# cgranerob/Land-Surface-Temperature-Super-Resolution-with-a-Scale-Invariance-Free-Neural-Approach

Hardware: AMD Instinct MI355X
Metric: LST+NDVI 256x256 patches/sec (train fwd+bwd), whole job (higher is better)
Workload: dtype f32; 1 GPU; ModelB SIF-NN-SR2 (gradFTM loss) batch 64/GPU, synthetic 256x256, 1x MI355X, fwd+loss+bwd+Adam; batch_per_gpu=64, patch=256x256 (LST 64x64 + NDVI 256x256), parallelism=dp1, loss=sr2

## Files before the change

land-surface-temperature-super-resolution-with-a-scale-invariance-free-neural-approach_amd/csrc/bn.hip:

```cpp
#include "edge_conv.h"

namespace {

template <int NT>
static __device__ __forceinline__ void block_sum2(double& s1, double& s2, double (*wsum)[2]) {
#pragma unroll
  for (int m = 32; m > 0; m >>= 1) { s1 += __shfl_xor(s1, m); s2 += __shfl_xor(s2, m); }
  const int lane = threadIdx.x & 63, wave = threadIdx.x >> 6;
  if (lane == 0) { wsum[wave][0] = s1; wsum[wave][1] = s2; }
  __syncthreads();
  s1 = 0.0; s2 = 0.0;
#pragma unroll
  for (int w = 0; w < NT / 64; ++w) { s1 += wsum[w][0]; s2 += wsum[w][1]; }
}

static __device__ __forceinline__ float mul2_add(float a, float b, float c, float d) {
#pragma clang fp contract(off)
  const float p = a * b, q = c * d;
  return p + q;
}

__global__ __launch_bounds__(256) void bn_finalize_kernel(const float* __restrict__ partials, int nblk, int C,
                                                          double count, const float* __restrict__ gamma,
                                                          const float* __restrict__ beta, float* run_mean,
// ... 173 lines not shown
      double t = 0.0;
      for (int g = 0; g < 64; ++g) t += part[g][el];
      xs_out[e] = poisoned != 0 ? __uint_as_float(0x7fc00000u) : (float)t;
    }
    return;
  }
  double s1 = 0.0, s2 = 0.0;
  for (int k = tid; k < nblk; k += 256) {
    const float2 v = *reinterpret_cast<const float2*>(partials + ((size_t)k * C + c) * 2);
    s1 += (double)v.x; s2 += (double)v.y;
  }
  block_sum2<256>(s1, s2, wsum);
  if (tid == 0) {
    const double db = s1, dg = s2;
    dbeta[c] = (float)db;
    dgamma[c] = (float)dg;
    write_coef<FROZEN>(coef, C, c, scale, mean, invstd, db, dg, count);
    write_coef_f<FROZEN>(coef_f, C, c, scale, shift, invstd, beta, db, dg, count);
    if (poisoned != 0) poison_channel(dgamma, dbeta, coef, coef_f, C, c);
  }
}

template <int NT, bool FROZEN>
__global__ __launch_bounds__(NT) void bn_bwd_finalize2_kernel(const float* __restrict__ pa, int na,
                                                               const float* __restrict__ pb, int nb, int C, double count,
                                                               const float* __restrict__ scale,
                                                               const float* __restrict__ mean,
                                                               const float* __restrict__ invstd, float* dgamma,
                                                               float* dbeta, double* coef, const float* __restrict__ shift,
                                                               const float* __restrict__ beta, float* coef_f, const int* nf) {
  SIFSR_CHAIN_PRIO();
  __shared__ double wsum[NT / 64][2];
  const int c = blockIdx.x, tid = threadIdx.x;
  const int poisoned = nf != nullptr ? nf[NF_BATCH] : 0;
  double s1 = 0.0, s2 = 0.0;
  for (int k = tid; k < na; k += NT) { const float2 v = *reinterpret_cast<const float2*>(pa + ((size_t)k * C + c) * 2); s1 += (double)v.x; s2 += (double)v.y; }
  for (int k = tid; k < nb; k += NT) { const float2 v = *reinterpret_cast<const float2*>(pb + ((size_t)k * C + c) * 2); s1 += (double)v.x; s2 += (double)v.y; }
  block_sum2<NT>(s1, s2, wsum);
  if (tid == 0) {
    const double db = s1;
    const double dg = (double)invstd[c] * (s2 - (double)mean[c] * db);
    dbeta[c] = (float)db;
    dgamma[c] = (float)dg;
    write_coef<FROZEN>(coef, C, c, scale, mean, invstd, db, dg, count);
    write_coef_f<FROZEN>(coef_f, C, c, scale, shift, invstd, beta, db, dg, count);
    if (poisoned != 0) poison_channel(dgamma, dbeta, coef, coef_f, C, c);
  }
}

template <int C, bool HS>
__global__ __launch_bounds__(256) void bn_bwd_apply_kernel(const float* __restrict__ g, const float* __restrict__ y,
                                                           const float* __restrict__ scale,
                                                           const float* __restrict__ shift,
                                                           const double* __restrict__ coef,
                                                           size_t nquads, float* __restrict__ dy, const PoolAdj pa) {
  SIFSR_CHAIN_PRIO();
  constexpr int Q = C / 4;
  const int c4 = threadIdx.x % Q;
  const float4 sc = ld4(scale + 4 * c4), sh = ld4(shift + 4 * c4);
  double sd[4], k1[4], k0[4];
// ... 65 lines not shown
    default: return SIFSR_ERR_SHAPE;
  }
  SIFSR_LAUNCH_CHECK();
  return SIFSR_OK;
}

int launch_bn_bwd_finalize(const float* partials, int nblk, int C, double count, const float* scale, const float* mean,
                           const float* invstd, float* dgamma, float* dbeta, double* coef, hipStream_t s, const float* shift,
                           const float* beta, float* coef_f, const float* xs_partials, int xs_n, float* xs_out, int frozen,
                           const int* nf) {
  if (coef_f != nullptr && (!shift || !beta)) return SIFSR_ERR_ARG;
  if (xs_partials != nullptr && (xs_n < 1 || !xs_out)) return SIFSR_ERR_ARG;
  const int extra = xs_partials != nullptr ? (xs_n + 3) / 4 : 0;
  if (frozen)
    hipLaunchKernelGGL(bn_bwd_finalize_kernel<true>, dim3(C + extra), dim3(256), 0, s, partials, nblk, C, count, scale, mean, invstd,
                       dgamma, dbeta, coef, shift, beta, coef_f, xs_partials, xs_n, xs_out, nf);
  else
    hipLaunchKernelGGL(bn_bwd_finalize_kernel<false>, dim3(C + extra), dim3(256), 0, s, partials, nblk, C, count, scale, mean, invstd,
                       dgamma, dbeta, coef, shift, beta, coef_f, xs_partials, xs_n, xs_out, nf);
  SIFSR_LAUNCH_CHECK();
  return SIFSR_OK;
}

int launch_bn_bwd_finalize2(const float* pa, int na, const float* pb, int nb, int C, double count, const float* scale,
                            const float* mean, const float* invstd, float* dgamma, float* dbeta, double* coef, hipStream_t s,
                            const float* shift, const float* beta, float* coef_f, int frozen, const int* nf) {
  if (coef_f != nullptr && (!shift || !beta)) return SIFSR_ERR_ARG;
#define BN_FIN2(NT_, FR_) hipLaunchKernelGGL((bn_bwd_finalize2_kernel<NT_, FR_>), dim3(C), dim3(NT_), 0, s, pa, na, pb, nb, C, count, scale, mean, \
                                             invstd, dgamma, dbeta, coef, shift, beta, coef_f, nf)
  if (na + nb > 4096) { if (frozen) BN_FIN2(1024, true); else BN_FIN2(1024, false); }
  else { if (frozen) BN_FIN2(256, true); else BN_FIN2(256, false); }
#undef BN_FIN2
  SIFSR_LAUNCH_CHECK();
  return SIFSR_OK;
}

int launch_bn_bwd_apply(const float* g, const float* y, const float* scale, const float* shift, const double* coef,
                        int C, size_t npix, float* dy, hipStream_t s, const float* gp, int H, int W) {
  if (gp != nullptr && (H < 2 || W < 2 || H % 2 || W % 2 || npix % ((size_t)H * W))) return SIFSR_ERR_SHAPE;
  const PoolAdj pa{gp, H, W};
  const size_t nquads = npix * (size_t)C / 4;
  size_t blocks = (nquads + 255) / 256;
  if (blocks > 8192) blocks = 8192;
  const bool hs = sifsr_half_storage();
#define BN_APPLY(C_, HS_) hipLaunchKernelGGL((bn_bwd_apply_kernel<C_, HS_>), dim3((int)blocks), dim3(256), 0, s, g, y, scale, shift, coef, nquads, dy, pa)
  switch (C) {
    case 16: if (hs) BN_APPLY(16, true); else BN_APPLY(16, false); break;
    case 32: if (hs) BN_APPLY(32, true); else BN_APPLY(32, false); break;
    case 64: if (hs) BN_APPLY(64, true); else BN_APPLY(64, false); break;
    default: return SIFSR_ERR_SHAPE;
  }
// ... 11 lines not shown
```

land-surface-temperature-super-resolution-with-a-scale-invariance-free-neural-approach_amd/csrc/edge_conv.h:

```cpp
#pragma once
#include "common.h"

int conv_in_fwd_blocks(int B, int H, int W);
int launch_conv_in_fwd(const float* x, const float* w, float* y, float* partials, int B, int H, int W, hipStream_t s,
                       int* nf_image = nullptr);
int launch_conv_in_wgrad(const float* x, const float* dy, float* partials, int nblk, float* dw, int B, int H, int W, hipStream_t s);
int launch_conv_out_fwd(const float* y, const float* scale, const float* shift, const float* w, const float* bias,
                        float* out, int B, int H, int W, hipStream_t s,
                        const int* nf = nullptr);
int launch_conv_out_dgrad(const float* dsr, const float* w, float* g, int B, int H, int W, hipStream_t s);
int launch_conv_out_wgrad(const float* y, const float* scale, const float* shift, const float* dsr, float* partials,
                          int nblk, float* dw, float* db, int B, int H, int W, hipStream_t s);
int launch_conv_in_wgrad_fused(const float* x, const float* g, const float* y, const float* scale, const float* shift,
                               const double* coef, float* partials, int nblk, float* dw, int B, int H, int W, hipStream_t s);
size_t conv_in_gram_scratch_floats();
int launch_conv_in_gram(const float* x, float* scratch, int B, int H, int W, hipStream_t s);
const double* conv_in_gram_result(const float* scratch);
int launch_conv_in_dz_wgrad(const float* x, const float* dz, float* partials, int nblk, int B, int H, int W, hipStream_t s);
int launch_conv_in_dw_combine(const float* partials, int nblk, const double* gram, const float* w, const double* coef, float* dw,
                              hipStream_t s);
int launch_tail_bwd_reduce(const float* y, const float* scale, const float* shift, const float* mean, const float* invstd,
                           const float* dsr, const float* w, float* wpart, float* bnpart, int nblk, int B, int H, int W,
                           hipStream_t s, int* nf = nullptr);
int launch_tail_bwd_apply(const float* y, const float* scale, const float* shift, const double* coef, const float* dsr,
                          const float* w, float* dy, int B, int H, int W, hipStream_t s);
int launch_sum_partials(const float* partials, int nblk, int n, float* out, hipStream_t s);

int launch_bn_finalize(const float* partials, int nblk, int C, double count, const float* gamma, const float* beta,
                       float* run_mean, float* run_var, float momentum, float eps, float* mean, float* invstd,
                       float* scale, float* shift, hipStream_t s,
                       int* nf = nullptr);
int launch_bn_eval_coeffs(const float* params, const float* running, float eps, float* scale, float* shift, hipStream_t s,
                          int* nf = nullptr, const int* nf_pack = nullptr);
int launch_bn_bwd_reduce(const float* g, const float* y, const float* scale, const float* shift, const float* mean,
                         const float* invstd, int C, size_t npix, float* partials, int nblk, hipStream_t s,
                         const float* gp = nullptr, int H = 0, int W = 0, float* g_out = nullptr);
int launch_bn_bwd_finalize(const float* partials, int nblk, int C, double count, const float* scale, const float* mean,
                           const float* invstd, float* dgamma, float* dbeta, double* coef, hipStream_t s,
                           const float* shift = nullptr, const float* beta = nullptr, float* coef_f = nullptr,
                           const float* xs_partials = nullptr, int xs_n = 0, float* xs_out = nullptr,
                           int frozen = 0,
                           const int* nf = nullptr);
int launch_bn_bwd_finalize2(const float* pa, int na, const float* pb, int nb, int C, double count, const float* scale,
                            const float* mean, const float* invstd, float* dgamma, float* dbeta, double* coef, hipStream_t s,
                            const float* shift = nullptr, const float* beta = nullptr, float* coef_f = nullptr, int frozen = 0,
                            const int* nf = nullptr);
int launch_bn_bwd_apply(const float* g, const float* y, const float* scale, const float* shift, const double* coef,
                        int C, size_t npix, float* dy, hipStream_t s, const float* gp = nullptr, int H = 0, int W = 0);
int launch_nbt_increment(long long* nbt, int n, hipStream_t s);

int launch_bn_frozen_stats(const float* running, float eps, float* mean, float* invstd, hipStream_t s);
int launch_conv_in_dgrad(const float* g, const float* y, const float* scale, const float* shift, const double* coef, const float* w,
                         float* dx, int B, int H, int W, hipStream_t s);

int launch_bnrelu_pool2(const float* y, const float* scale, const float* shift, float* out, int B, int H, int W, int C, hipStream_t s);
int launch_bnrelu_add(const float* p, const float* y, const float* scale, const float* shift, float* out, int C, size_t npix, hipStream_t s);
int launch_bnrelu_up2x(const float* y, const float* scale, const float* shift, float* out, int B, int Hin, int Win, int C, hipStream_t s);
int launch_pool2_bwd(const float* gp, float* g, int B, int H, int W, int C, int accumulate, hipStream_t s);
int launch_up2x_bwd(const float* gu, float* g, int B, int Hin, int Win, int C, hipStream_t s, const float* bn_y = nullptr,
                    const float* bn_scale = nullptr, const float* bn_shift = nullptr, float* bn_partials = nullptr);
int up2x_bwd_stat_rows(int B, int Hin, int Win, int C);

int launch_adam_flat(float* p, const float* g, float* m, float* v, int n, float lr, float beta1, float beta2, float eps,
                     float weight_decay, int step, float grad_scale, hipStream_t s);

int launch_adam_flat_dev(float* p, const float* g, float* m, float* v, int n, float lr, float beta1, float beta2, float eps,
                         float weight_decay, long long* step_dev, float* coef2, float grad_scale, hipStream_t s);

int launch_tiles_prepare(const float* lst, const float* ndvi, float* x, int T, int tiles_x, int win, long long lst_step_y,
                         long long lst_step_x, int lst_row, long long ndvi_step_y, long long ndvi_step_x, int ndvi_row,
                         float mean_lst, float std_lst, float mean_ndvi, float std_ndvi, int clip_ndvi, hipStream_t s);
int launch_tiles_paste(const float* sr, float* out, int T, int tiles_x, int hr, long long out_row, float mean, float std,
                       hipStream_t s);
int launch_l4pool4(const float* x, float* out, int B, int H, int W, hipStream_t s);
size_t psnr_ssim_scratch_bytes(int B, int H, int W);
int launch_psnr_ssim(const float* pred, const float* targ, int B, int H, int W, void* scratch, float* out2, hipStream_t s);
size_t psnr_ssim_masked_scratch_bytes(int B, int H, int W);
int launch_psnr_ssim_masked(const float* pred, const float* targ, const unsigned char* valid, int scale, int B, int H, int W,
                            void* scratch, float* out2, int* counts2, hipStream_t s);

size_t eval_metrics_scratch_bytes(int B, int H, int W);
int launch_eval_metrics(const float* a, const float* b, int B, int H, int W, const float* taps9, float data_range,
                        void* scratch, double* out8, hipStream_t s);
// ... 9 lines not shown
```

land-surface-temperature-super-resolution-with-a-scale-invariance-free-neural-approach_amd/csrc/engine.hip:

```cpp
#include "engine.h"
#include "switches.h"

#include <stdio.h>
#include <stdlib.h>

#include <mutex>
#include <vector>

static thread_local bool t_half_storage = false;
bool sifsr_half_storage() { return t_half_storage; }
HalfStorageScope::HalfStorageScope(bool on) : prev(t_half_storage) { t_half_storage = on; }
HalfStorageScope::~HalfStorageScope() { t_half_storage = prev; }

static int env_int(const char* name, int dflt) { const char* v = getenv(name); return v ? atoi(v) : dflt; }
const Switches& sifsr_switches() {
  static const Switches sw = {
      env_int("SIFSR_WGRAD_STREAM", 1), env_int("SIFSR_WGRAD_WINO", 2),  env_int("SIFSR_NO_WINO", 0),
      env_int("SIFSR_NO_WINO8", 0),     env_int("SIFSR_NO_BWD16", 0),    env_int("SIFSR_TAIL_APPLY", 0),
      env_int("SIFSR_HEAD_LINEAR", 0),  env_int("SIFSR_BF16_BWD16", 0),  env_int("SIFSR_DBG_EARLY_REDUCE", 3),
      env_int("SIFSR_DBG_POOL_ON_LOAD", 1)};
  return sw;
}

static constexpr int enc_prev[3] = {L_IN3, L_D1C, L_D2C};
// ... 125 lines not shown
  int lvW(int lv) const { return W >> lv; }
  float* f(size_t off) const { return ws + off; }
  float* y(int l) const { return ws + lay.y[l]; }
  float* g(int l) const { return ws + lay.g[l]; }
  float* mean(int l) const { return ws + lay.mean + nt.L[l].ch_off; }
  float* invstd(int l) const { return ws + lay.invstd + nt.L[l].ch_off; }
  float* scale(int l) const { return ws + lay.scale + nt.L[l].ch_off; }
  float* shift(int l) const { return ws + lay.shift + nt.L[l].ch_off; }
  float* coef_f(int l) const { return ws + lay.coef_f + 4 * (size_t)nt.L[l].ch_off; }
  double* coef() const { return reinterpret_cast<double*>(ws + lay.coef); }
  float* slab(int l) const { return ws + lay.slab_l[l]; }
  int* nf() const { return reinterpret_cast<int*>(ws + lay.nf); }
  size_t wn(int l) const { return (size_t)9 * nt.L[l].cin * nt.L[l].cout; }
  const float* w_dgrad_f32(int l) const { return ws + lay.wdg + 4 * (size_t)nt.L[l].wpack_off; }
  const float* w_fwd(int l) const { return bf16 ? w_dgrad_f32(l) + wn(l) : ws + lay.wfwd + nt.L[l].wpack_off; }
  const float* w_dgrad(int l) const { return bf16 ? w_dgrad_f32(l) + wn(l) + wn(l) / 2 : w_dgrad_f32(l); }
  const float* w_fwd_wino(int l) const { return ws + lay.wwf + (size_t)nt.L[l].wpack_off / 9 * 16; }
  const float* w_dgrad_wino(int l) const { return ws + lay.wwd + (size_t)nt.L[l].wpack_off / 9 * 16; }
};

struct BwdState {
  WgradReduceJob jobs[16];
  int njobs = 0;
  int last_fused = -1;
};

ConvSrc src_raw(const float* p, int C) { ConvSrc s; s.ptr = p; s.scale = nullptr; s.shift = nullptr; s.C = C; s.coff = 0; s.nq = C / 16; return s; }
ConvSrc src_act(const Ctx& c, int l) {
  ConvSrc s; s.ptr = c.y(l); s.scale = c.scale(l); s.shift = c.shift(l); s.C = c.nt.L[l].cout; s.coff = 0; s.nq = s.C / 16; return s;
}
ConvSrc src_none() { ConvSrc s; s.ptr = nullptr; s.scale = nullptr; s.shift = nullptr; s.C = 0; s.coff = 0; s.nq = 0; return s; }

#define SIFSR_TRY(expr) do { int rc__ = (expr); if (rc__ != SIFSR_OK) return rc__; } while (0)

struct SideLane {
  hipStream_t s = nullptr;
  hipEvent_t ev[SIFSR_NUM_BN_LAYERS] = {};
  hipEvent_t join = nullptr;
  hipEvent_t aux = nullptr;
  bool ok = false;
  std::mutex in_use;
};

int g_side_override = -1;

SideLane* side_lane(hipStream_t main_stream) {
  if (!(g_side_override >= 0 ? g_side_override : sifsr_switches().wgrad_stream)) return nullptr;
  static std::mutex mu;
  static SideLane lanes[16];
  static bool tried[16] = {};
  int dev = 0;
  if (hipGetDevice(&dev) != hipSuccess || dev < 0 || dev >= 16) return nullptr;
  hipStreamCaptureStatus cap = hipStreamCaptureStatusNone;
  if (hipStreamIsCapturing(main_stream, &cap) != hipSuccess) { (void)hipGetLastError(); return nullptr; }
  if (cap != hipStreamCaptureStatusNone) return nullptr;
  if (main_stream != nullptr) {
    hipDevice_t sdev = -1;
    if (hipStreamGetDevice(main_stream, &sdev) != hipSuccess || (int)sdev != dev) { (void)hipGetLastError(); return nullptr; }
  }
  std::lock_guard<std::mutex> lk(mu);
  SideLane& L = lanes[dev];
  if (!tried[dev]) {
    tried[dev] = true;
    int lo = 0, hi = 0;
    (void)hipDeviceGetStreamPriorityRange(&lo, &hi);
    bool ok = hipStreamCreateWithPriority(&L.s, hipStreamNonBlocking, lo) == hipSuccess;
    for (int i = 0; ok && i < SIFSR_NUM_BN_LAYERS; ++i) ok = hipEventCreateWithFlags(&L.ev[i], hipEventDisableTiming) == hipSuccess;
    ok = ok && hipEventCreateWithFlags(&L.join, hipEventDisableTiming) == hipSuccess;
    ok = ok && hipEventCreateWithFlags(&L.aux, hipEventDisableTiming) == hipSuccess;
    L.ok = ok;
    (void)hipGetLastError();
  }
  return L.ok ? &L : nullptr;
}

struct SideLaneGuard {
  SideLane* lane; hipStream_t main; bool forked = false, joined = false;
  SideLaneGuard(SideLane* l, hipStream_t m) : lane(l), main(m) { if (lane) lane->in_use.lock(); }
  int join() {
    if (!lane || joined) return SIFSR_OK;
    joined = true;
    if (!forked) return SIFSR_OK;
    if (hipEventRecord(lane->join, lane->s) != hipSuccess || hipStreamWaitEvent(main, lane->join, 0) != hipSuccess) return SIFSR_ERR_ARG;
    return SIFSR_OK;
  }
  ~SideLaneGuard() { if (lane) { (void)join(); lane->in_use.unlock(); } }
};

constexpr int PROF_SLOTS = 24;
constexpr size_t PROF_POOL = 1024;
struct ProfSlot {
  int layer = -1, phase = 0;
// ... 44 lines not shown
  a.dst[1] = a.dst[0];
  a.bf16 = c.bf16;
  a.wpack = c.w_fwd(l);
  a.wpack_wino = c.w_fwd_wino(l);
  a.addend = nullptr; a.addC = 0;
  a.stat_partials = training ? c.f(c.lay.partials) : nullptr;
  a.dst_split = L.cout / 16;
  a.B = c.B; a.H = c.lvH(L.level); a.W = c.lvW(L.level);
  a.NQ = L.cin / 16;
  {
    ProfScope ps(l, 1, c.s);
    SIFSR_TRY(launch_conv3x3_mfma(a, L.cout, 0, c.s));
  }
  if (training)
    SIFSR_TRY(bn_unit_finalize(c, l, conv3x3_grid_blocks(c.B, a.H, a.W, L.cout, conv3x3_wino_kind(a, L.cout, 0)), running, momentum, eps));
  return SIFSR_OK;
}

int bn_bwd_reduce_blocks(size_t npix) {
  const size_t nb = npix / 256;
  return (int)(nb > 1024 ? 1024 : (nb < 1 ? 1 : nb));
}
int bn_unit_bwd(const Ctx& c, int l, const float* gp = nullptr, int fused_stats = 0, int border_rows = -1,
                bool writeback = true) {
  const LayerInfo& L = c.nt.L[l];
  const int lh = c.lvH(L.level), lw = c.lvW(L.level);
  const size_t npix = c.lay.npix[L.level];
  float* dgamma = c.grads + L.gamma_off, *dbeta = c.grads + L.beta_off;
  if (fused_stats > 0) {
    if (gp != nullptr) return SIFSR_ERR_ARG;
    return launch_bn_bwd_finalize2(c.f(c.lay.partials), fused_stats, c.f(c.lay.bpart), border_rows >= 0 ? border_rows : dgrad_border_waves(c.B, lh, lw, 16),
                                   L.cout, (double)npix, c.scale(l), c.mean(l), c.invstd(l), dgamma, dbeta, c.coef(), c.s, c.shift(l),
                                   c.params + L.beta_off, c.coef_f(l), c.frozen, c.nf());
  }
  const int nblk = bn_bwd_reduce_blocks(npix);
  SIFSR_TRY(launch_bn_bwd_reduce(c.g(l), c.y(l), c.scale(l), c.shift(l), c.mean(l), c.invstd(l), L.cout, npix, c.f(c.lay.partials), nblk,
                                 c.s, gp, lh, lw, (gp && writeback) ? c.g(l) : nullptr));
  return launch_bn_bwd_finalize(c.f(c.lay.partials), nblk, L.cout, (double)npix, c.scale(l), c.mean(l), c.invstd(l), dgamma, dbeta,
                                c.coef(), c.s, c.shift(l), c.params + L.beta_off, c.coef_f(l), nullptr, 0, nullptr, c.frozen, c.nf());
}

static bool wgrad_wino_policy(int cout) {
  const int mode = sifsr_switches().wgrad_wino;
  return mode == 2 || (mode == 1 && cout <= 32);
}

int conv_unit_wgrad(const Ctx& c, int l, ConvSrc s0, ConvSrc s1, const float* dy, bool dy_stored = false) {
  const LayerInfo& L = c.nt.L[l];
  WgradArgs a;
  a.src[0] = s0; a.src[1] = s1;
  a.dy = dy; a.slabs = c.slab(l);
  if (!dy_stored) { a.dy_y = c.y(l); a.dy_coef = c.coef_f(l); }
  a.B = c.B; a.H = c.lvH(L.level); a.W = c.lvW(L.level);
  a.NQ = L.cin / 16;
  a.ntiles = c.B * ((a.H + 7) / 8) * ((a.W + 15) / 16);
  a.bf16 = c.bf16;
  const bool wino = wgrad_wino_policy(L.cout) && conv3x3_wgrad_use_wino(a, L.cin, L.cout);
  const int nbi = wino ? wgrad_wino_nbi_chunk(L.cin) : wgrad_nbi_chunk(a, L.cin);
  const int nblk = wgrad_blocks(L.cin, L.cout, L.cin / (16 * nbi), a.ntiles, wino);
  if ((size_t)nblk * (L.cin / (16 * nbi)) * 9 * (16 * nbi) * L.cout > c.lay.slab_cap[l]) return SIFSR_ERR_WORKSPACE;
  hipStream_t ws = c.s;
  if (c.side != nullptr) {
    if (hipEventRecord(c.side->ev[l], c.s) != hipSuccess || hipStreamWaitEvent(c.side->s, c.side->ev[l], 0) != hipSuccess)
      return SIFSR_ERR_ARG;
    ws = c.side->s;
    *c.forked = true;
  }
  {
    ProfScope ps(l, 3, ws);
    if (wino) SIFSR_TRY(launch_conv3x3_wgrad_wino(a, L.cin, L.cout, nblk, ws));
    else SIFSR_TRY(launch_conv3x3_wgrad(a, L.cin, L.cout, nblk, ws));
  }
  WgradReduceJob& j = c.bwd->jobs[c.bwd->njobs++];
  j.slab_off = c.lay.slab_l[l]; j.nblk = nblk; j.cin = L.cin; j.cout = L.cout; j.nbi_chunk = nbi; j.w_off = L.w_off;
  return SIFSR_OK;
}

int conv_unit_dgrad(const Ctx& c, int l, const float* dy, float* g0, int C0, int split_ch, float* g1, int C1,
                    const float* addend, int bn_layer = -1, int* stat_rows = nullptr, bool dy_stored = false) {
  const LayerInfo& L = c.nt.L[l];
  const bool fuse = bn_layer >= 0 && L.cin == 16 && C0 == 16 && split_ch == 16 && g1 == nullptr && addend == nullptr &&
                    c.nt.L[bn_layer].cout == 16 && c.nt.L[bn_layer].level == L.level;
  if (stat_rows) *stat_rows = 0;
  ConvArgs a;
  a.src[0] = src_raw(dy, L.cout); a.src[1] = src_none();
  const float* dy_edge = dy;
  if (!dy_stored) {
    a.bw_y = c.y(l); a.bw_coef = c.coef_f(l); a.bw_border = c.f(c.lay.dy_border);
    dy_edge = a.bw_border;
// ... 45 lines not shown
  else a.g = dy;
  if (!dy_stored) { a.y = c.y(l); a.coef = c.coef_f(l); a.dy_border = c.f(c.lay.dy_border); }
  a.wpack_wino = c.w_dgrad_wino(l);
  a.gin = gin; a.addend = addend;
  if (fuse) {
    a.bn_y = c.y(bn_layer); a.bn_scale = c.scale(bn_layer); a.bn_shift = c.shift(bn_layer); a.stat_partials = c.f(c.lay.partials);
    if (stat_rows) *stat_rows = grid;
  }
  a.slabs = c.slab(l);
  a.B = c.B; a.H = lh; a.W = lw;
  a.half = c.bf16;
  if (store_dz && !fuse) return SIFSR_ERR_ARG;
  a.store_dz = store_dz ? 1 : 0;
  a.pool_gp = pool_gp;
  {
    ProfScope ps(l, 2, c.s);
    SIFSR_TRY(launch_conv3x3_bwd16(a, c.s));
  }
  SIFSR_TRY(launch_dgrad_border_fix(dy_stored ? dy : a.dy_border, 16, c.w_dgrad_f32(l), 16, gin, 16, 16, gin, 16, c.B, lh, lw, c.s, c.bf16,
                                    fuse ? a.bn_y : nullptr, fuse ? a.bn_scale : nullptr, fuse ? a.bn_shift : nullptr,
                                    fuse ? c.f(c.lay.bpart) : nullptr, a.store_dz));
  WgradReduceJob& j = c.bwd->jobs[c.bwd->njobs++];
  j.slab_off = c.lay.slab_l[l]; j.nblk = grid; j.cin = 16; j.cout = 16; j.nbi_chunk = 1; j.w_off = L.w_off;
  if (c.side != nullptr && hipEventRecord(c.side->ev[l], c.s) != hipSuccess) return SIFSR_ERR_ARG;
  c.bwd->last_fused = l;
  *applied = true;
  return SIFSR_OK;
}

int conv_unit_bwd(const Ctx& c, int l, ConvSrc s0, const float* dy, float* gin, const float* addend, int bn_layer, int* stat_rows,
                  int dy_mode = 1) {
  bool fused = false;
  SIFSR_TRY(conv_unit_bwd16(c, l, s0, dy, gin, addend, bn_layer, stat_rows, dy_mode, &fused));
  if (fused) return SIFSR_OK;
  const int cin = c.nt.L[l].cin;
  SIFSR_TRY(conv_unit_wgrad(c, l, s0, src_none(), dy, dy_mode == 0));
  return conv_unit_dgrad(c, l, dy, gin, cin, cin, nullptr, 0, addend, bn_layer, stat_rows, dy_mode == 0);
}

int finish_wgrads(const Ctx& c, hipStream_t st) {
  BwdState& b = *c.bwd;
  if (b.njobs > 0) SIFSR_TRY(launch_wgrad_reduce_batched(c.ws, b.jobs, b.njobs, c.grads, st));
  b.njobs = 0;
  return SIFSR_OK;
}
int finish_wgrads_side(const Ctx& c) {
  if (c.bwd->last_fused >= 0) {
    if (hipStreamWaitEvent(c.side->s, c.side->ev[c.bwd->last_fused], 0) != hipSuccess) return SIFSR_ERR_ARG;
    *c.forked = true;
  }
  return finish_wgrads(c, c.side->s);
}

}

int sifsr_engine_forward(const float* x, float* sr, const float* params, float* running, long long* nbt, float* ws,
                         size_t ws_floats, int B, int H, int W, int training, float momentum, float eps,
                         hipStream_t s, int bf16) {
  if (!x || !sr || !params || !running || !ws) return SIFSR_ERR_ARG;
  Ctx c{sifsr_net(), WsLayout(), ws, params, B, H, W, s};
  if (bf16 < 0 || bf16 > 1) return SIFSR_ERR_ARG;
  c.bf16 = bf16;
  const HalfStorageScope storage(bf16 == 1);
  SIFSR_TRY(sifsr_layout(B, H, W, training, &c.lay));
  if (ws_floats < c.lay.fwd_end) return SIFSR_ERR_WORKSPACE;
  const NetTable& nt = c.nt;
  const WsLayout& w = c.lay;

  SIFSR_TRY(launch_pack_weights(params, c.f(w.wfwd), c.f(w.wdg), s, c.f(w.wwf), c.f(w.wwd), training ? nbt : nullptr, SIFSR_NUM_BN_LAYERS,
                                c.nf(), NF_IMAGE + B));
  if (!training) {
    SIFSR_TRY(launch_bn_eval_coeffs(params, running, eps, c.f(w.scale), c.f(w.shift), s, c.nf(), c.nf() + NF_IMAGE + B));
  }
// ... 40 lines not shown
                          size_t ws_floats, int B, int H, int W, hipStream_t s, int bf16, int frozen, float* dx) {
  if (!x || !dsr || !params || !grads || !ws) return SIFSR_ERR_ARG;
  Ctx c{sifsr_net(), WsLayout(), ws, params, B, H, W, s};
  if (bf16 < 0 || bf16 > 1) return SIFSR_ERR_ARG;
  if ((frozen != 0 || dx != nullptr) && bf16 != 0) return SIFSR_ERR_ARG;
  c.bf16 = bf16;
  c.frozen = frozen != 0;
  const HalfStorageScope storage(bf16 == 1);
  SIFSR_TRY(sifsr_layout(B, H, W, 1, &c.lay));
  if (ws_floats < c.lay.total) return SIFSR_ERR_WORKSPACE;
  const NetTable& nt = c.nt;
  const WsLayout& w = c.lay;
  const Switches& sw = sifsr_switches();
  BwdState state;
  c.grads = grads; c.bwd = &state;
  c.side = (size_t)B * H * W >= 2u * 65536u || g_side_override == 1 ? side_lane(s) : nullptr;
  SideLaneGuard lane_guard(c.side, s);
  c.forked = &lane_guard.forked;

  const bool head_linear = sw.head_linear != 0 && dx == nullptr && bwd16_usable(c, L_IN3, src_act(c, L_IN0));
  if (head_linear) {
    hipStream_t gs = s;
    if (c.side != nullptr) {
      if (hipEventRecord(c.side->ev[L_IN0], s) != hipSuccess || hipStreamWaitEvent(c.side->s, c.side->ev[L_IN0], 0) != hipSuccess) return SIFSR_ERR_ARG;
      lane_guard.forked = true;
      gs = c.side->s;
    }
    SIFSR_TRY(launch_conv_in_gram(x, c.f(w.gram), B, H, W, gs));
    if (c.side != nullptr && hipEventRecord(c.side->aux, gs) != hipSuccess) return SIFSR_ERR_ARG;
  }
  const bool tail_in_bwd16 = !sw.tail_apply && bwd16_usable(c, L_U3B, src_act(c, L_U3A));
  {
    const LayerInfo& L = nt.L[L_U3B];
    int nblk = B * ((H + 15) / 16) * ((W + 15) / 16);
    if (nblk > 768) nblk = 768;
    SIFSR_TRY(launch_tail_bwd_reduce(c.y(L_U3B), c.scale(L_U3B), c.shift(L_U3B), c.mean(L_U3B), c.invstd(L_U3B), dsr,
                                     params + nt.out_w_off, c.f(w.slabs), c.f(w.partials), nblk, B, H, W, s, c.nf()));
    if (grads + nt.out_b_off != grads + nt.out_w_off + 144) return SIFSR_ERR_ARG;
    SIFSR_TRY(launch_bn_bwd_finalize(c.f(w.partials), nblk, 16, (double)w.npix[0], c.scale(L_U3B), c.mean(L_U3B), c.invstd(L_U3B),
                                     grads + L.gamma_off, grads + L.beta_off, c.coef(), s, c.shift(L_U3B), params + L.beta_off,
                                     c.coef_f(L_U3B), c.f(w.slabs), 145, grads + nt.out_w_off, c.frozen, c.nf()));
    if (!tail_in_bwd16)
      SIFSR_TRY(launch_tail_bwd_apply(c.y(L_U3B), c.scale(L_U3B), c.shift(L_U3B), c.coef(), dsr, params + nt.out_w_off, c.g(L_U3B),
                                      B, H, W, s));
  }

  int up_rows = 0;
  for (int k = 2; k >= 0; --k) {
    const int lv = 2 - k;
    const int la = dec_a[k], lb = dec_b[k], ls = dec_skip[k], ll = dec_low[k];
    if (k != 2) SIFSR_TRY(bn_unit_bwd(c, lb, nullptr, up_rows, 0));
    int rows_a = 0;
    SIFSR_TRY(conv_unit_bwd(c, lb, src_act(c, la), k == 2 && tail_in_bwd16 ? dsr : c.g(lb), c.g(la), nullptr, la, &rows_a,
                            k == 2 ? (tail_in_bwd16 ? 2 : 0) : 1));
    SIFSR_TRY(bn_unit_bwd(c, la, nullptr, rows_a));
    SIFSR_TRY(conv_unit_wgrad(c, la, src_raw(c.f(w.U[k]), uc[k]), src_act(c, ls), c.g(la)));
    SIFSR_TRY(conv_unit_dgrad(c, la, c.g(la), c.f(w.gU[k]), uc[k], uc[k], c.g(ls), nt.L[ls].cout, nullptr));
    up_rows = up2x_bwd_stat_rows(B, c.lvH(lv + 1), c.lvW(lv + 1), uc[k]);
    if ((size_t)up_rows * uc[k] * 2 > w.partials_cap) up_rows = 0;
    SIFSR_TRY(launch_up2x_bwd(c.f(w.gU[k]), c.g(ll), B, c.lvH(lv + 1), c.lvW(lv + 1), uc[k], s,
                              up_rows ? c.y(ll) : nullptr, up_rows ? c.scale(ll) : nullptr, up_rows ? c.shift(ll) : nullptr,
                              up_rows ? c.f(w.partials) : nullptr));
  }

  for (int k = 2; k >= 0; --k) {
    const int la = enc_a[k], lb = enc_b[k], lc = enc_c[k];
    const int er = sw.early_reduce;
    if (c.side != nullptr && (er == 3 || (er == 2 && k != 1) || (er == 1 && k == 0))) SIFSR_TRY(finish_wgrads_side(c));
    SIFSR_TRY(bn_unit_bwd(c, lc, k < 2 ? c.f(w.gP[k + 1]) : nullptr, k == 2 ? up_rows : 0, 0));
    SIFSR_TRY(conv_unit_wgrad(c, lc, src_raw(c.f(w.R[k]), pc[k]), src_none(), c.g(lc)));
    int rows_b = 0, rows_a = 0;
    SIFSR_TRY(conv_unit_dgrad(c, lc, c.g(lc), c.g(lb), pc[k], pc[k], nullptr, 0, nullptr, lb, &rows_b));
    SIFSR_TRY(bn_unit_bwd(c, lb, nullptr, rows_b));
    SIFSR_TRY(conv_unit_bwd(c, lb, src_act(c, la), c.g(lb), c.g(la), nullptr, la, &rows_a));
    SIFSR_TRY(bn_unit_bwd(c, la, nullptr, rows_a));
    SIFSR_TRY(conv_unit_bwd(c, la, src_raw(c.f(w.P[k]), pc[k]), c.g(la), c.f(w.gP[k]), c.g(lb), -1, nullptr));
  }

  const bool pool_on_load = sw.pool_on_load != 0 && bwd16_usable(c, L_IN3, src_act(c, L_IN0));
  SIFSR_TRY(bn_unit_bwd(c, L_IN3, c.f(w.gP[0]), 0, -1, !pool_on_load));
  int rows_in0 = 0;
  bool fused_in3 = false;
  SIFSR_TRY(conv_unit_bwd16(c, L_IN3, src_act(c, L_IN0), c.g(L_IN3), c.g(L_IN0), nullptr, L_IN0, &rows_in0, 1, &fused_in3, head_linear,
                            pool_on_load ? c.f(w.gP[0]) : nullptr));
  if (pool_on_load && !fused_in3) return SIFSR_ERR_ARG;
  if (head_linear && !fused_in3) return SIFSR_ERR_ARG;
  if (!fused_in3) SIFSR_TRY(conv_unit_wgrad(c, L_IN3, src_act(c, L_IN0), src_none(), c.g(L_IN3)));
  if (c.side != nullptr) SIFSR_TRY(finish_wgrads_side(c));
  if (!fused_in3) SIFSR_TRY(conv_unit_dgrad(c, L_IN3, c.g(L_IN3), c.g(L_IN0), 16, 16, nullptr, 0, nullptr, L_IN0, &rows_in0));
  {
    const LayerInfo& L = nt.L[L_IN0];
    if (rows_in0 > 0) {
// ... 76 lines not shown
```

land-surface-temperature-super-resolution-with-a-scale-invariance-free-neural-approach_amd/csrc/resample.hip:

```cpp
#include "edge_conv.h"

namespace {

__device__ __forceinline__ float4 maybe_bnrelu(float4 v, const float* scale, const float* shift, int c) {
  return scale != nullptr ? bn_relu4(v, ld4(scale + c), ld4(shift + c)) : v;
}

template <bool HS>
__global__ void bnrelu_pool2_kernel(const float* __restrict__ y, const float* scale, const float* shift,
                                    float* __restrict__ out, int B, int H, int W, int C) {
  const unsigned Q = C / 4, Ho = H / 2, Wo = W / 2;
  const unsigned n = (unsigned)B * Ho * Wo * Q;
  for (unsigned e = blockIdx.x * blockDim.x + threadIdx.x; e < n; e += gridDim.x * blockDim.x) {
    const unsigned p = e / Q;
    const int c = (int)(e - p * Q) * 4;
    const unsigned rr = p / Wo, ox = p - rr * Wo, b = rr / Ho, oy = rr - b * Ho;
    const size_t s = (((size_t)b * H + 2 * oy) * W + 2 * ox) * C + c;
    const float4 v00 = maybe_bnrelu(ldA4<HS>(y, s), scale, shift, c), v01 = maybe_bnrelu(ldA4<HS>(y, s + C), scale, shift, c);
    const float4 v10 = maybe_bnrelu(ldA4<HS>(y, s + (size_t)W * C), scale, shift, c);
    const float4 v11 = maybe_bnrelu(ldA4<HS>(y, s + (size_t)W * C + C), scale, shift, c);
    float4 o;
    o.x = (v00.x + v01.x + v10.x + v11.x) * 0.25f;
    o.y = (v00.y + v01.y + v10.y + v11.y) * 0.25f;
    o.z = (v00.z + v01.z + v10.z + v11.z) * 0.25f;
// ... 133 lines not shown
  for (int e = tid; e < 256 * Q; e += 256) {
    const int c4 = e % Q, p = e / Q;
    const int oy = oy0 + (p >> 4), ox = ox0 + (p & 15);
    if (oy >= Ho || ox >= Wo) continue;
    int y0, y1, x0, x1; float hy0, hy1, hx0, hx1;
    up_coord(oy, Hin, Ho, y0, y1, hy0, hy1);
    up_coord(ox, Win, Wo, x0, x1, hx0, hx1);
    const float4 v00 = src[((y0 - sy0) * SR + (x0 - sx0)) * Q + c4], v01 = src[((y0 - sy0) * SR + (x1 - sx0)) * Q + c4];
    const float4 v10 = src[((y1 - sy0) * SR + (x0 - sx0)) * Q + c4], v11 = src[((y1 - sy0) * SR + (x1 - sx0)) * Q + c4];
    float4 o;
    o.x = hy0 * (hx0 * v00.x + hx1 * v01.x) + hy1 * (hx0 * v10.x + hx1 * v11.x);
    o.y = hy0 * (hx0 * v00.y + hx1 * v01.y) + hy1 * (hx0 * v10.y + hx1 * v11.y);
    o.z = hy0 * (hx0 * v00.z + hx1 * v01.z) + hy1 * (hx0 * v10.z + hx1 * v11.z);
    o.w = hy0 * (hx0 * v00.w + hx1 * v01.w) + hy1 * (hx0 * v10.w + hx1 * v11.w);
    stA4<HS>(out, ((size_t)(b * Ho + oy) * Wo + ox) * C + 4 * c4, o);
  }
}

template <int C, bool HS>
__global__ __launch_bounds__(256) void up2x_bwd_tile_kernel(const float* __restrict__ gu, float* __restrict__ g, int Hin,
                                                            int Win, const float* __restrict__ bn_y,
                                                            const float* __restrict__ bn_scale,
                                                            const float* __restrict__ bn_shift,
                                                            float* __restrict__ bn_partials) {
  SIFSR_CHAIN_PRIO();
  constexpr int TL = 8, HR = 2 * TL + 3, NCH = C / 16;
  __shared__ float4 hi[HR * HR * 4];
  __shared__ float4 tmp[HR * TL * 4];
  __shared__ float wxs[TL][5], wys[TL][5];
  const int tid = threadIdx.x;
  const int Ho = 2 * Hin, Wo = 2 * Win;
  const int ix0 = blockIdx.x * TL, iy0 = blockIdx.y * TL;
  const int b = blockIdx.z / NCH, ch0 = (blockIdx.z % NCH) * 16;
  if (tid < 2 * TL * 5) {
    const bool isy = tid >= TL * 5;
    const int t = isy ? tid - TL * 5 : tid;
    const int il = t / 5, k = t - il * 5;
    const int i = (isy ? iy0 : ix0) + il, in = isy ? Hin : Win, on = isy ? Ho : Wo;
    const int o = 2 * i - 2 + k;
    float w = 0.f;
    if (i < in && o >= 0 && o < on) {
      int a0, a1; float l0, l1;
      up_coord(o, in, on, a0, a1, l0, l1);
      w = (a0 == i ? l0 : 0.f) + (a1 == i ? l1 : 0.f);
    }
    if (isy) wys[il][k] = w; else wxs[il][k] = w;
  }
// ... 40 lines not shown
        const float4 sc = ld4(bn_scale + ch0 + 4 * q), sh = ld4(bn_shift + ch0 + 4 * q);
        d1.x = fmaf(yv.x, sc.x, sh.x) > 0.f ? acc.x : 0.f; d2.x = d1.x * yv.x;
        d1.y = fmaf(yv.y, sc.y, sh.y) > 0.f ? acc.y : 0.f; d2.y = d1.y * yv.y;
        d1.z = fmaf(yv.z, sc.z, sh.z) > 0.f ? acc.z : 0.f; d2.z = d1.z * yv.z;
        d1.w = fmaf(yv.w, sc.w, sh.w) > 0.f ? acc.w : 0.f; d2.w = d1.w * yv.w;
      }
      float v8[8] = {d1.x, d1.y, d1.z, d1.w, d2.x, d2.y, d2.z, d2.w};
#pragma unroll
      for (int m = 4; m < 64; m <<= 1)
#pragma unroll
        for (int j = 0; j < 8; ++j) v8[j] += __shfl_xor(v8[j], m);
      __syncthreads();
      float* const red = reinterpret_cast<float*>(hi);
      if ((tid & 63) < 4) {
#pragma unroll
        for (int j = 0; j < 8; ++j) red[((tid >> 6) * 4 + (tid & 3)) * 8 + j] = v8[j];
      }
      __syncthreads();
      if (tid < 32) {
        const int qq = tid & 3, r = (tid >> 2) & 3, which = tid >> 4;
        const float sum = (red[(0 * 4 + qq) * 8 + which * 4 + r] + red[(1 * 4 + qq) * 8 + which * 4 + r]) +
                          (red[(2 * 4 + qq) * 8 + which * 4 + r] + red[(3 * 4 + qq) * 8 + which * 4 + r]);
        const size_t row = ((size_t)b * gridDim.y + blockIdx.y) * gridDim.x + blockIdx.x;
        bn_partials[(row * C + ch0 + 4 * qq + r) * 2 + which] = sum;
      }
    }
  }
}

inline int grid_for(size_t n) {
  size_t b = (n + 255) / 256;
  return (int)(b > 16384 ? 16384 : (b < 1 ? 1 : b));
}

}

int launch_bnrelu_pool2(const float* y, const float* scale, const float* shift, float* out, int B, int H, int W, int C, hipStream_t s) {
  if (H % 2 || W % 2 || C % 4 || (size_t)B * H * W * C >= ((size_t)1 << 32)) return SIFSR_ERR_SHAPE;
  if (sifsr_half_storage()) hipLaunchKernelGGL(bnrelu_pool2_kernel<true>, dim3(grid_for((size_t)B * H / 2 * W / 2 * C / 4)), dim3(256), 0, s, y, scale, shift, out, B, H, W, C);
  else hipLaunchKernelGGL(bnrelu_pool2_kernel<false>, dim3(grid_for((size_t)B * H / 2 * W / 2 * C / 4)), dim3(256), 0, s, y, scale, shift, out, B, H, W, C);
  SIFSR_LAUNCH_CHECK();
  return SIFSR_OK;
}
int launch_bnrelu_add(const float* p, const float* y, const float* scale, const float* shift, float* out, int C, size_t npix, hipStream_t s) {
  if (C % 4) return SIFSR_ERR_SHAPE;
  const size_t nq = npix * C / 4;
  if (sifsr_half_storage()) hipLaunchKernelGGL(bnrelu_add_kernel<true>, dim3(grid_for(nq)), dim3(256), 0, s, p, y, scale, shift, out, C, nq);
// ... 12 lines not shown
    else { if (hs) SIFSR_UP(64, true); else SIFSR_UP(64, false); }
#undef SIFSR_UP
    SIFSR_LAUNCH_CHECK();
    return SIFSR_OK;
  }
  if (sifsr_half_storage()) hipLaunchKernelGGL(bnrelu_up2x_kernel<true>, dim3(grid_for((size_t)B * Hin * Win * C)), dim3(256), 0, s, y, scale, shift, out, B, Hin, Win, C);
  else hipLaunchKernelGGL(bnrelu_up2x_kernel<false>, dim3(grid_for((size_t)B * Hin * Win * C)), dim3(256), 0, s, y, scale, shift, out, B, Hin, Win, C);
  SIFSR_LAUNCH_CHECK();
  return SIFSR_OK;
}
int launch_pool2_bwd(const float* gp, float* g, int B, int H, int W, int C, int accumulate, hipStream_t s) {
  if (H % 2 || W % 2 || C % 4) return SIFSR_ERR_SHAPE;
  if (sifsr_half_storage()) hipLaunchKernelGGL(pool2_bwd_kernel<true>, dim3(grid_for((size_t)B * H * W * C / 4)), dim3(256), 0, s, gp, g, B, H, W, C, accumulate);
  else hipLaunchKernelGGL(pool2_bwd_kernel<false>, dim3(grid_for((size_t)B * H * W * C / 4)), dim3(256), 0, s, gp, g, B, H, W, C, accumulate);
  SIFSR_LAUNCH_CHECK();
  return SIFSR_OK;
}
int up2x_bwd_stat_rows(int B, int Hin, int Win, int C) {
  if (!((C == 16 || C == 32 || C == 64) && (size_t)B * (C / 16) <= 65535)) return 0;
  return B * ((Hin + 7) / 8) * ((Win + 7) / 8);
}

int launch_up2x_bwd(const float* gu, float* g, int B, int Hin, int Win, int C, hipStream_t s, const float* bn_y,
                    const float* bn_scale, const float* bn_shift, float* bn_partials) {
  if (C % 4) return SIFSR_ERR_SHAPE;
  if (bn_partials != nullptr && (!bn_y || !bn_scale || !bn_shift || up2x_bwd_stat_rows(B, Hin, Win, C) == 0)) return SIFSR_ERR_ARG;
  if ((C == 16 || C == 32 || C == 64) && (size_t)B * (C / 16) <= 65535) {
    const dim3 grid((Win + 7) / 8, (Hin + 7) / 8, B * (C / 16));
#define SIFSR_UPB(CV, HV) hipLaunchKernelGGL((up2x_bwd_tile_kernel<CV, HV>), grid, dim3(256), 0, s, gu, g, Hin, Win, bn_y, bn_scale, bn_shift, bn_partials)
    const bool hs = sifsr_half_storage();
    if (C == 16) { if (hs) SIFSR_UPB(16, true); else SIFSR_UPB(16, false); }
    else if (C == 32) { if (hs) SIFSR_UPB(32, true); else SIFSR_UPB(32, false); }
    else { if (hs) SIFSR_UPB(64, true); else SIFSR_UPB(64, false); }
#undef SIFSR_UPB
    SIFSR_LAUNCH_CHECK();
    return SIFSR_OK;
  }
  if (sifsr_half_storage()) hipLaunchKernelGGL(up2x_bwd_kernel<true>, dim3(grid_for((size_t)B * Hin * Win * C / 4)), dim3(256), 0, s, gu, g, B, Hin, Win, C);
  else hipLaunchKernelGGL(up2x_bwd_kernel<false>, dim3(grid_for((size_t)B * Hin * Win * C / 4)), dim3(256), 0, s, gu, g, B, Hin, Win, C);
  SIFSR_LAUNCH_CHECK();
  return SIFSR_OK;
}
```

Measured before the change: 10710 patches/s.

## Store up2x-bwd BN partials channel-major and batch side-lane event handoffs

```diff
diff --git a/land-surface-temperature-super-resolution-with-a-scale-invariance-free-neural-approach_amd/csrc/bn.hip b/land-surface-temperature-super-resolution-with-a-scale-invariance-free-neural-approach_amd/csrc/bn.hip
--- a/land-surface-temperature-super-resolution-with-a-scale-invariance-free-neural-approach_amd/csrc/bn.hip
+++ b/land-surface-temperature-super-resolution-with-a-scale-invariance-free-neural-approach_amd/csrc/bn.hip
@@ -219,8 +219,8 @@
 }
 
 template <int NT, bool FROZEN>
-__global__ __launch_bounds__(NT) void bn_bwd_finalize2_kernel(const float* __restrict__ pa, int na,
-                                                               const float* __restrict__ pb, int nb, int C, double count,
+__global__ __launch_bounds__(NT) void bn_bwd_finalize2_kernel(const float* __restrict__ pa, int na, PartialLayout la,
+                                                               const float* __restrict__ pb, int nb, PartialLayout lb, int C, double count,
                                                                const float* __restrict__ scale,
                                                                const float* __restrict__ mean,
                                                                const float* __restrict__ invstd, float* dgamma,
@@ -231,8 +231,9 @@
   const int c = blockIdx.x, tid = threadIdx.x;
   const int poisoned = nf != nullptr ? nf[NF_BATCH] : 0;
   double s1 = 0.0, s2 = 0.0;
-  for (int k = tid; k < na; k += NT) { const float2 v = *reinterpret_cast<const float2*>(pa + ((size_t)k * C + c) * 2); s1 += (double)v.x; s2 += (double)v.y; }
-  for (int k = tid; k < nb; k += NT) { const float2 v = *reinterpret_cast<const float2*>(pb + ((size_t)k * C + c) * 2); s1 += (double)v.x; s2 += (double)v.y; }
+  pa += (size_t)c * la.chan * 2; pb += (size_t)c * lb.chan * 2;
+  for (int k = tid; k < na; k += NT) { const float2 v = *reinterpret_cast<const float2*>(pa + (size_t)k * la.row * 2); s1 += (double)v.x; s2 += (double)v.y; }
+  for (int k = tid; k < nb; k += NT) { const float2 v = *reinterpret_cast<const float2*>(pb + (size_t)k * lb.row * 2); s1 += (double)v.x; s2 += (double)v.y; }
   block_sum2<NT>(s1, s2, wsum);
   if (tid == 0) {
     const double db = s1;
@@ -344,11 +345,12 @@
   return SIFSR_OK;
 }
 
-int launch_bn_bwd_finalize2(const float* pa, int na, const float* pb, int nb, int C, double count, const float* scale,
-                            const float* mean, const float* invstd, float* dgamma, float* dbeta, double* coef, hipStream_t s,
-                            const float* shift, const float* beta, float* coef_f, int frozen, const int* nf) {
+int launch_bn_bwd_finalize2(const float* pa, int na, PartialLayout la, const float* pb, int nb, PartialLayout lb, int C, double count,
+                            const float* scale, const float* mean, const float* invstd, float* dgamma, float* dbeta, double* coef,
+                            hipStream_t s, const float* shift, const float* beta, float* coef_f, int frozen, const int* nf) {
   if (coef_f != nullptr && (!shift || !beta)) return SIFSR_ERR_ARG;
-#define BN_FIN2(NT_, FR_) hipLaunchKernelGGL((bn_bwd_finalize2_kernel<NT_, FR_>), dim3(C), dim3(NT_), 0, s, pa, na, pb, nb, C, count, scale, mean, \
+  if (la.row < 1 || la.chan < 1 || lb.row < 1 || lb.chan < 1) return SIFSR_ERR_ARG;
+#define BN_FIN2(NT_, FR_) hipLaunchKernelGGL((bn_bwd_finalize2_kernel<NT_, FR_>), dim3(C), dim3(NT_), 0, s, pa, na, la, pb, nb, lb, C, count, scale, mean, \
                                              invstd, dgamma, dbeta, coef, shift, beta, coef_f, nf)
   if (na + nb > 4096) { if (frozen) BN_FIN2(1024, true); else BN_FIN2(1024, false); }
   else { if (frozen) BN_FIN2(256, true); else BN_FIN2(256, false); }
diff --git a/land-surface-temperature-super-resolution-with-a-scale-invariance-free-neural-approach_amd/csrc/edge_conv.h b/land-surface-temperature-super-resolution-with-a-scale-invariance-free-neural-approach_amd/csrc/edge_conv.h
--- a/land-surface-temperature-super-resolution-with-a-scale-invariance-free-neural-approach_amd/csrc/edge_conv.h
+++ b/land-surface-temperature-super-resolution-with-a-scale-invariance-free-neural-approach_amd/csrc/edge_conv.h
@@ -41,10 +41,11 @@
                            const float* xs_partials = nullptr, int xs_n = 0, float* xs_out = nullptr,
                            int frozen = 0,
                            const int* nf = nullptr);
-int launch_bn_bwd_finalize2(const float* pa, int na, const float* pb, int nb, int C, double count, const float* scale,
-                            const float* mean, const float* invstd, float* dgamma, float* dbeta, double* coef, hipStream_t s,
-                            const float* shift = nullptr, const float* beta = nullptr, float* coef_f = nullptr, int frozen = 0,
-                            const int* nf = nullptr);
+struct PartialLayout { int row, chan; };
+int launch_bn_bwd_finalize2(const float* pa, int na, PartialLayout la, const float* pb, int nb, PartialLayout lb, int C, double count,
+                            const float* scale, const float* mean, const float* invstd, float* dgamma, float* dbeta, double* coef,
+                            hipStream_t s, const float* shift = nullptr, const float* beta = nullptr, float* coef_f = nullptr,
+                            int frozen = 0, const int* nf = nullptr);
 int launch_bn_bwd_apply(const float* g, const float* y, const float* scale, const float* shift, const double* coef,
                         int C, size_t npix, float* dy, hipStream_t s, const float* gp = nullptr, int H = 0, int W = 0);
 int launch_nbt_increment(long long* nbt, int n, hipStream_t s);
@@ -58,7 +59,8 @@
 int launch_bnrelu_up2x(const float* y, const float* scale, const float* shift, float* out, int B, int Hin, int Win, int C, hipStream_t s);
 int launch_pool2_bwd(const float* gp, float* g, int B, int H, int W, int C, int accumulate, hipStream_t s);
 int launch_up2x_bwd(const float* gu, float* g, int B, int Hin, int Win, int C, hipStream_t s, const float* bn_y = nullptr,
-                    const float* bn_scale = nullptr, const float* bn_shift = nullptr, float* bn_partials = nullptr);
+                    const float* bn_scale = nullptr, const float* bn_shift = nullptr, float* bn_partials = nullptr,
+                    bool partials_channel_major = false);
 int up2x_bwd_stat_rows(int B, int Hin, int Win, int C);
 
 int launch_adam_flat(float* p, const float* g, float* m, float* v, int n, float lr, float beta1, float beta2, float eps,
diff --git a/land-surface-temperature-super-resolution-with-a-scale-invariance-free-neural-approach_amd/csrc/engine.hip b/land-surface-temperature-super-resolution-with-a-scale-invariance-free-neural-approach_amd/csrc/engine.hip
--- a/land-surface-temperature-super-resolution-with-a-scale-invariance-free-neural-approach_amd/csrc/engine.hip
+++ b/land-surface-temperature-super-resolution-with-a-scale-invariance-free-neural-approach_amd/csrc/engine.hip
@@ -171,7 +171,8 @@
 struct BwdState {
   WgradReduceJob jobs[16];
   int njobs = 0;
-  int last_fused = -1;
+  bool fused_unpublished = false;
+  int nhand = 0;
 };
 
 ConvSrc src_raw(const float* p, int C) { ConvSrc s; s.ptr = p; s.scale = nullptr; s.shift = nullptr; s.C = C; s.coff = 0; s.nq = C / 16; return s; }
@@ -184,7 +185,8 @@
 
 struct SideLane {
   hipStream_t s = nullptr;
-  hipEvent_t ev[SIFSR_NUM_BN_LAYERS] = {};
+  static constexpr int NEV = 24;
+  hipEvent_t ev[NEV] = {};
   hipEvent_t join = nullptr;
   hipEvent_t aux = nullptr;
   bool ok = false;
@@ -214,9 +216,14 @@
     int lo = 0, hi = 0;
     (void)hipDeviceGetStreamPriorityRange(&lo, &hi);
     bool ok = hipStreamCreateWithPriority(&L.s, hipStreamNonBlocking, lo) == hipSuccess;
-    for (int i = 0; ok && i < SIFSR_NUM_BN_LAYERS; ++i) ok = hipEventCreateWithFlags(&L.ev[i], hipEventDisableTiming) == hipSuccess;
+    auto lane_event = [](hipEvent_t* e) {
+      if (hipEventCreateWithFlags(e, hipEventDisableTiming | hipEventDisableSystemFence) == hipSuccess) return true;
+      (void)hipGetLastError();
+      return hipEventCreateWithFlags(e, hipEventDisableTiming) == hipSuccess;
+    };
+    for (int i = 0; ok && i < SideLane::NEV; ++i) ok = lane_event(&L.ev[i]);
     ok = ok && hipEventCreateWithFlags(&L.join, hipEventDisableTiming) == hipSuccess;
-    ok = ok && hipEventCreateWithFlags(&L.aux, hipEventDisableTiming) == hipSuccess;
+    ok = ok && lane_event(&L.aux);
     L.ok = ok;
     (void)hipGetLastError();
   }
@@ -307,15 +314,18 @@
   return (int)(nb > 1024 ? 1024 : (nb < 1 ? 1 : nb));
 }
 int bn_unit_bwd(const Ctx& c, int l, const float* gp = nullptr, int fused_stats = 0, int border_rows = -1,
-                bool writeback = true) {
+                bool writeback = true,
+                bool from_up = false) {
   const LayerInfo& L = c.nt.L[l];
   const int lh = c.lvH(L.level), lw = c.lvW(L.level);
   const size_t npix = c.lay.npix[L.level];
   float* dgamma = c.grads + L.gamma_off, *dbeta = c.grads + L.beta_off;
   if (fused_stats > 0) {
     if (gp != nullptr) return SIFSR_ERR_ARG;
-    return launch_bn_bwd_finalize2(c.f(c.lay.partials), fused_stats, c.f(c.lay.bpart), border_rows >= 0 ? border_rows : dgrad_border_waves(c.B, lh, lw, 16),
-                                   L.cout, (double)npix, c.scale(l), c.mean(l), c.invstd(l), dgamma, dbeta, c.coef(), c.s, c.shift(l),
+    const PartialLayout row_major{L.cout, 1}, chan_major{1, fused_stats};
+    return launch_bn_bwd_finalize2(c.f(c.lay.partials), fused_stats, from_up ? chan_major : row_major, c.f(c.lay.bpart),
+                                   border_rows >= 0 ? border_rows : dgrad_border_waves(c.B, lh, lw, 16), row_major, L.cout,
+                                   (double)npix, c.scale(l), c.mean(l), c.invstd(l), dgamma, dbeta, c.coef(), c.s, c.shift(l),
                                    c.params + L.beta_off, c.coef_f(l), c.frozen, c.nf());
   }
   const int nblk = bn_bwd_reduce_blocks(npix);
@@ -328,6 +338,16 @@
 static bool wgrad_wino_policy(int cout) {
   const int mode = sifsr_switches().wgrad_wino;
   return mode == 2 || (mode == 1 && cout <= 32);
+}
+
+int lane_handoff(const Ctx& c) {
+  BwdState& b = *c.bwd;
+  if (b.nhand >= SideLane::NEV) return SIFSR_ERR_ARG;
+  const hipEvent_t e = c.side->ev[b.nhand++];
+  if (hipEventRecord(e, c.s) != hipSuccess || hipStreamWaitEvent(c.side->s, e, 0) != hipSuccess) return SIFSR_ERR_ARG;
+  b.fused_unpublished = false;
+  *c.forked = true;
+  return SIFSR_OK;
 }
 
 int conv_unit_wgrad(const Ctx& c, int l, ConvSrc s0, ConvSrc s1, const float* dy, bool dy_stored = false) {
@@ -346,10 +366,8 @@
   if ((size_t)nblk * (L.cin / (16 * nbi)) * 9 * (16 * nbi) * L.cout > c.lay.slab_cap[l]) return SIFSR_ERR_WORKSPACE;
   hipStream_t ws = c.s;
   if (c.side != nullptr) {
-    if (hipEventRecord(c.side->ev[l], c.s) != hipSuccess || hipStreamWaitEvent(c.side->s, c.side->ev[l], 0) != hipSuccess)
-      return SIFSR_ERR_ARG;
+    SIFSR_TRY(lane_handoff(c));
     ws = c.side->s;
-    *c.forked = true;
   }
   {
     ProfScope ps(l, 3, ws);
@@ -441,8 +459,7 @@
                                     fuse ? c.f(c.lay.bpart) : nullptr, a.store_dz));
   WgradReduceJob& j = c.bwd->jobs[c.bwd->njobs++];
   j.slab_off = c.lay.slab_l[l]; j.nblk = grid; j.cin = 16; j.cout = 16; j.nbi_chunk = 1; j.w_off = L.w_off;
-  if (c.side != nullptr && hipEventRecord(c.side->ev[l], c.s) != hipSuccess) return SIFSR_ERR_ARG;
-  c.bwd->last_fused = l;
+  c.bwd->fused_unpublished = c.side != nullptr;
   *applied = true;
   return SIFSR_OK;
 }
@@ -464,10 +481,9 @@
   return SIFSR_OK;
 }
 int finish_wgrads_side(const Ctx& c) {
-  if (c.bwd->last_fused >= 0) {
-    if (hipStreamWaitEvent(c.side->s, c.side->ev[c.bwd->last_fused], 0) != hipSuccess) return SIFSR_ERR_ARG;
-    *c.forked = true;
-  }
+  if (c.bwd->njobs == 0) return SIFSR_OK;
+  if (c.bwd->fused_unpublished) SIFSR_TRY(lane_handoff(c));
+  *c.forked = true;
   return finish_wgrads(c, c.side->s);
 }
 
@@ -554,8 +570,7 @@
   if (head_linear) {
     hipStream_t gs = s;
     if (c.side != nullptr) {
-      if (hipEventRecord(c.side->ev[L_IN0], s) != hipSuccess || hipStreamWaitEvent(c.side->s, c.side->ev[L_IN0], 0) != hipSuccess) return SIFSR_ERR_ARG;
-      lane_guard.forked = true;
+      SIFSR_TRY(lane_handoff(c));
       gs = c.side->s;
     }
     SIFSR_TRY(launch_conv_in_gram(x, c.f(w.gram), B, H, W, gs));
@@ -581,7 +596,7 @@
   for (int k = 2; k >= 0; --k) {
     const int lv = 2 - k;
     const int la = dec_a[k], lb = dec_b[k], ls = dec_skip[k], ll = dec_low[k];
-    if (k != 2) SIFSR_TRY(bn_unit_bwd(c, lb, nullptr, up_rows, 0));
+    if (k != 2) SIFSR_TRY(bn_unit_bwd(c, lb, nullptr, up_rows, 0, true, true));
     int rows_a = 0;
     SIFSR_TRY(conv_unit_bwd(c, lb, src_act(c, la), k == 2 && tail_in_bwd16 ? dsr : c.g(lb), c.g(la), nullptr, la, &rows_a,
                             k == 2 ? (tail_in_bwd16 ? 2 : 0) : 1));
@@ -592,14 +607,14 @@
     if ((size_t)up_rows * uc[k] * 2 > w.partials_cap) up_rows = 0;
     SIFSR_TRY(launch_up2x_bwd(c.f(w.gU[k]), c.g(ll), B, c.lvH(lv + 1), c.lvW(lv + 1), uc[k], s,
                               up_rows ? c.y(ll) : nullptr, up_rows ? c.scale(ll) : nullptr, up_rows ? c.shift(ll) : nullptr,
-                              up_rows ? c.f(w.partials) : nullptr));
+                              up_rows ? c.f(w.partials) : nullptr, true));
   }
 
   for (int k = 2; k >= 0; --k) {
     const int la = enc_a[k], lb = enc_b[k], lc = enc_c[k];
     const int er = sw.early_reduce;
     if (c.side != nullptr && (er == 3 || (er == 2 && k != 1) || (er == 1 && k == 0))) SIFSR_TRY(finish_wgrads_side(c));
-    SIFSR_TRY(bn_unit_bwd(c, lc, k < 2 ? c.f(w.gP[k + 1]) : nullptr, k == 2 ? up_rows : 0, 0));
+    SIFSR_TRY(bn_unit_bwd(c, lc, k < 2 ? c.f(w.gP[k + 1]) : nullptr, k == 2 ? up_rows : 0, 0, true, k == 2));
     SIFSR_TRY(conv_unit_wgrad(c, lc, src_raw(c.f(w.R[k]), pc[k]), src_none(), c.g(lc)));
     int rows_b = 0, rows_a = 0;
     SIFSR_TRY(conv_unit_dgrad(c, lc, c.g(lc), c.g(lb), pc[k], pc[k], nullptr, 0, nullptr, lb, &rows_b));
diff --git a/land-surface-temperature-super-resolution-with-a-scale-invariance-free-neural-approach_amd/csrc/resample.hip b/land-surface-temperature-super-resolution-with-a-scale-invariance-free-neural-approach_amd/csrc/resample.hip
--- a/land-surface-temperature-super-resolution-with-a-scale-invariance-free-neural-approach_amd/csrc/resample.hip
+++ b/land-surface-temperature-super-resolution-with-a-scale-invariance-free-neural-approach_amd/csrc/resample.hip
@@ -179,7 +179,7 @@
                                                             int Win, const float* __restrict__ bn_y,
                                                             const float* __restrict__ bn_scale,
                                                             const float* __restrict__ bn_shift,
-                                                            float* __restrict__ bn_partials) {
+                                                            float* __restrict__ bn_partials, int part_cm) {
   SIFSR_CHAIN_PRIO();
   constexpr int TL = 8, HR = 2 * TL + 3, NCH = C / 16;
   __shared__ float4 hi[HR * HR * 4];
@@ -266,7 +266,8 @@
         const float sum = (red[(0 * 4 + qq) * 8 + which * 4 + r] + red[(1 * 4 + qq) * 8 + which * 4 + r]) +
                           (red[(2 * 4 + qq) * 8 + which * 4 + r] + red[(3 * 4 + qq) * 8 + which * 4 + r]);
         const size_t row = ((size_t)b * gridDim.y + blockIdx.y) * gridDim.x + blockIdx.x;
-        bn_partials[(row * C + ch0 + 4 * qq + r) * 2 + which] = sum;
+        const size_t nrows = (size_t)(gridDim.z / NCH) * gridDim.y * gridDim.x, ch = ch0 + 4 * qq + r;
+        bn_partials[(part_cm ? ch * nrows + row : row * C + ch) * 2 + which] = sum;
       }
     }
   }
@@ -325,12 +326,13 @@
 }
 
 int launch_up2x_bwd(const float* gu, float* g, int B, int Hin, int Win, int C, hipStream_t s, const float* bn_y,
-                    const float* bn_scale, const float* bn_shift, float* bn_partials) {
+                    const float* bn_scale, const float* bn_shift, float* bn_partials, bool partials_channel_major) {
   if (C % 4) return SIFSR_ERR_SHAPE;
   if (bn_partials != nullptr && (!bn_y || !bn_scale || !bn_shift || up2x_bwd_stat_rows(B, Hin, Win, C) == 0)) return SIFSR_ERR_ARG;
   if ((C == 16 || C == 32 || C == 64) && (size_t)B * (C / 16) <= 65535) {
     const dim3 grid((Win + 7) / 8, (Hin + 7) / 8, B * (C / 16));
-#define SIFSR_UPB(CV, HV) hipLaunchKernelGGL((up2x_bwd_tile_kernel<CV, HV>), grid, dim3(256), 0, s, gu, g, Hin, Win, bn_y, bn_scale, bn_shift, bn_partials)
+#define SIFSR_UPB(CV, HV) hipLaunchKernelGGL((up2x_bwd_tile_kernel<CV, HV>), grid, dim3(256), 0, s, gu, g, Hin, Win, bn_y, bn_scale, bn_shift, bn_partials, \
+                                           partials_channel_major ? 1 : 0)
     const bool hs = sifsr_half_storage();
     if (C == 16) { if (hs) SIFSR_UPB(16, true); else SIFSR_UPB(16, false); }
     else if (C == 32) { if (hs) SIFSR_UPB(32, true); else SIFSR_UPB(32, false); }
```

Result: no change. 10800 patches/s, median of 6 (+0.9%).
